# soldasim/BOSS.jl

Measured on AMD Instinct MI355X. Metric: gp_posterior_updates_per_sec (+ acq_evals_per_sec), N=4096 d=8 fp64, higher is better.
Workload: dtype f64; 1 GPU; d=8 synthetic blackbox, GaussianProcess(Matern52) surrogate, N=4096 fp64 posterior update + ExpectedImprovement over 8192 candidates per GPU (BASELINE.json configs[1]+[2]); N=4096, d=8, M_per_gpu=8192, kernel=matern52, parallelism=single GPU: no exchange

## Files before the change

### boss.jl_amd/api.py

```python
from __future__ import annotations

import ctypes as C
import os
from typing import Optional, Sequence

import numpy as np

_HERE = os.path.dirname(os.path.abspath(__file__))
LIB_PATH = os.environ.get("BOSS_LIB_PATH") or os.path.join(_HERE, "libbosship.so")

BOSS_OK, BOSS_E_INVALID, BOSS_E_NO_DEVICE, BOSS_E_NOT_PD, BOSS_E_NEG_VAR, BOSS_E_NOT_FITTED, BOSS_E_ALLOC = range(7)
KERNELS = {"matern32": 0, "matern52": 1, "sqexp": 2}
FIT_NO_SYNC = 1

_c_dp = C.POINTER(C.c_double)
_c_ucp = C.POINTER(C.c_ubyte)

SIGNATURES = {
    "boss_version": (C.c_char_p, []),
    "boss_last_error": (C.c_char_p, []),
    "boss_device_count": (C.c_int, [C.POINTER(C.c_int)]),
    "boss_set_stream": (C.c_int, [C.c_int, C.c_void_p]),
    "boss_device_sync": (C.c_int, [C.c_int]),
    "boss_gp_create": (C.c_int, [C.c_int, C.c_int, C.c_int, C.c_int, _c_dp, _c_dp, _c_ucp, C.POINTER(C.c_void_p)]),
# ... 2283 lines not shown
    return ms.value, n.value


def _update_path(g: GP):
    lib = load_library()
    fn = lib.boss_debug_update_path
    fn.restype = C.c_int
    fn.argtypes = [C.c_void_p, C.POINTER(C.c_int), C.POINTER(C.c_int), C.POINTER(C.c_int)]
    ch, tm, fb = C.c_int(0), C.c_int(0), C.c_int(0)
    _check(fn(g._h, C.byref(ch), C.byref(tm), C.byref(fb)))
    return ch.value, tm.value, fb.value


def _append_path(g: GP) -> int:
    fn = load_library().boss_debug_append_path
    fn.restype = C.c_int
    fn.argtypes = [C.c_void_p, C.POINTER(C.c_int)]
    out = C.c_int(-1)
    _check(fn(g._h, C.byref(out)))
    return out.value


def _fallbacks(device: int = 0):
    lib = load_library()
    fn = lib.boss_debug_fallbacks
    fn.restype = C.c_int
    fn.argtypes = [C.c_int, C.POINTER(C.c_long), C.POINTER(C.c_int)]
    n, off = C.c_long(0), C.c_int(0)
    _check(fn(device, C.byref(n), C.byref(off)))
    return n.value, off.value


def _set_launches(device: int = 0):
    lib = load_library()
    fn = lib.boss_debug_set_launches
    fn.restype = C.c_int
    fn.argtypes = [C.c_int, C.POINTER(C.c_long), C.POINTER(C.c_long)]
    a, b = C.c_long(0), C.c_long(0)
    fn(device, C.byref(a), C.byref(b))
    return a.value, b.value


def _set_grad_launches(device: int = 0):
    lib = load_library()
    fn = lib.boss_debug_set_grad_launches
    fn.restype = C.c_int
    fn.argtypes = [C.c_int, C.POINTER(C.c_long)]
    a = C.c_long(0)
    fn(device, C.byref(a))
    return a.value


def _acq_path(device: int = 0):
    fn = load_library().boss_debug_acq_path
    fn.restype = C.c_int
    fn.argtypes = [C.c_int, C.POINTER(C.c_int)]
    out = (C.c_int * 5)()
    _check(fn(device, out))
    return tuple(out)


def _acq_prune_set(device: int = 0, min_tiles: int = -1, K: int = -1, s: int = -1, cap: int = -1, slack: Optional[float] = None):
    lib = load_library()
    fn = lib.boss_debug_acq_prune_set
    fn.restype = C.c_int
    fn.argtypes = [C.c_int] * 5
    _check(fn(device, int(min_tiles), int(K), int(s), int(cap)))
    if slack is not None:
        fs = lib.boss_debug_acq_prune_slack
        fs.restype = C.c_int
        fs.argtypes = [C.c_int, C.c_double]
        _check(fs(device, float(slack)))


def _acq_prune_bounds(M: int, device: int = 0):
    fn = load_library().boss_debug_acq_prune_bounds
    fn.restype = C.c_int
    fn.argtypes = [C.c_int, C.c_int, C.c_void_p, C.c_void_p, C.c_void_p]
    mua, vs, ub = np.zeros(M), np.zeros(M), np.zeros(M)
    _check(fn(device, int(M), mua.ctypes.data, vs.ctypes.data, ub.ctypes.data))
    return mua, vs, ub


def _acq_counters(g: GP):
    fn = load_library().boss_debug_acq_counters
    fn.restype = C.c_int
    fn.argtypes = [C.c_void_p, C.POINTER(C.c_long)]
    out = (C.c_long * 4)()
    _check(fn(g._h, out))
    return tuple(out)
```

### boss.jl_amd/csrc/bosship.hip

```cpp
#include "../../include/bosship.h"

#include <hip/hip_runtime.h>

#include <algorithm>
#include <cmath>
#include <cstdint>
#include <cstdio>
#include <cstdlib>
#include <atomic>
#include <chrono>
#include <cstring>
#include <functional>
#include <limits>
#include <map>
#include <mutex>
#include <string>
#include <thread>
#include <vector>

#include "gp_kernels.hpp"
#include "potrf.hpp"
#include "chain.hpp"
#include "small_calls.hpp"
#include "rider.hpp"
// ... 409 lines not shown
        hipEvent_t e;
        (void)hipEventCreate(&e);
        return e;
    }
};

struct boss_gpset {
    Ctx* ctx = nullptr;
    std::atomic<int> refs{0};
    void* slab = nullptr;
    void* host_block = nullptr;
    size_t slab_bytes = 0, host_bytes = 0;
};
static bool slab_cache_on() {
    static const bool v = !(getenv("BOSS_SLAB_CACHE") && atoi(getenv("BOSS_SLAB_CACHE")) == 0) &&
                          !poison_alloc();
    return v;
}
static void gpset_release_storage(boss_gpset* st) {
    Ctx* c = st->ctx;
    void *slab = st->slab, *hb = st->host_block;
    if (c && slab_cache_on()) {
        std::lock_guard<std::mutex> lk(c->slab_mtx);
        if (slab && st->slab_bytes > c->slab_cache_bytes) {
            std::swap(slab, c->slab_cache);
            c->slab_cache_bytes = st->slab_bytes;
        }
        if (hb && st->host_bytes > c->hostblk_cache_bytes) {
            std::swap(hb, c->hostblk_cache);
            c->hostblk_cache_bytes = st->host_bytes;
        }
    }
    if (slab) (void)hipFree(slab);
    if (hb) (void)hipHostFree(hb);
    st->slab = st->host_block = nullptr;
}

struct boss_gp {
    Ctx* ctx = nullptr;
    boss_gpset* set = nullptr;
    int kernel = 0, d = 0, N = 0, Np = 0, nblk = 0, ld = 0;
    double *Xraw = nullptr, *Xsc = nullptr, *y = nullptr, *mean = nullptr, *A = nullptr;
    double *LT = nullptr, *DT2 = nullptr, *avec = nullptr;
    bool have_lt = false;
    double *inv16 = nullptr, *Dinv = nullptr, *Dinv2 = nullptr, *hyp = nullptr, *invlam = nullptr, *scal = nullptr;
    int* info = nullptr;
    unsigned char* discrete_dev = nullptr;
    std::vector<unsigned char> discrete;
    double amp2 = 0.0;
    bool has_mean = false, fitted = false, pending = false, have_dinv = false;
    bool dinv_used = false;
    bool dinv_used_prev = false;
    bool gated = false;
    bool chained = false;
    bool fell_back = false;
    int trail_used = -1;
    double* host_res = nullptr;
    double* host_res_dev = nullptr;
    bool par_in_args = false;
    unsigned long long res_seq = 0;
    bool res_polled = false;
    double* host_par = nullptr;
    hipEvent_t par_ev = nullptr;
    unsigned long long epoch = 0;
    unsigned long long factor_gen = 0, dinv0_gen = ~0ull;
    hipEvent_t dinv_ev = nullptr;
    bool dinv_pending = false;
    bool aug = false;
    int npts = 0, ldx = 0, nhead = 0;
    bool gibbs = false;
    double *lamX = nullptr, *ampX = nullptr, *noiseX = nullptr;
    bool kprog = false;
    bool kgrad = false;
    FitProg* kp = nullptr;
    double *Winv = nullptr, *Linv = nullptr;
    double* W2 = nullptr;
    int w2_np = 0;
    unsigned long long w2_gen = ~0ull;
    bool w2_used = false;
    bool have_winv = false;
    int few_calls = 0;
    int append_calls = 0;
    double* prune_a = nullptr;
    int prune_a_np = 0;
    unsigned long long prune_a_gen = ~0ull;
    int prune_skip = 0, prune_backoff = 0;
    int append_path = 0;
};

struct boss_cand {
    Ctx* ctx = nullptr;
    int d = 0, M = 0, Mp = 0;
    double* Craw = nullptr;
};

struct boss_track {
    Ctx* ctx = nullptr;
    boss_gp* gp = nullptr;
    int d = 0, M = 0, Mp = 0, tiles = 0, Ncap = 0, N = 0;
    unsigned long long epoch = 0;
    double *V = nullptr, *Csc = nullptr, *mu = nullptr, *var = nullptr, *mean = nullptr;
    bool has_mean = false;
    bool gibbs = false;
    double *Clam = nullptr, *Camp = nullptr;
    bool aug = false;
};

static inline int round_up(int x, int m) { return (x + m - 1) / m * m; }
struct SetBatch {
    int nb = 1;
    size_t sA = 0, sInv16 = 0, sDinv = 0, sDinv2 = 0, sW = 0, sX = 0;
    size_t sPar = 0;
};
struct MeanFold {
    const double* J = nullptr;
    size_t sJ = 0;
    int T = 0;
    double* dmean = nullptr;
    double* dtheta = nullptr;
};
static void linv_enqueue(boss_gp* g, hipStream_t s, double* U, double* Lw, const SetBatch& B = SetBatch());
constexpr int MAX_ROWS = 46080;

extern "C" const char* boss_version(void) { return "bosship 0.1.0 (gfx950, fp64 MFMA)"; }
extern "C" const char* boss_last_error(void) { return g_last_error.c_str(); }

extern "C" int boss_device_count(int* n_out) {
    const int n = visible_devices();
    hipError_t e = n > 0 ? hipSuccess : hipErrorNoDevice;
    if (e != hipSuccess || n <= 0) {
        if (n_out) *n_out = 0;
        return fail(BOSS_E_NO_DEVICE, "no HIP device visible (bosship has no CPU fallback)");
    }
    if (n_out) *n_out = n;
    return BOSS_OK;
}

extern "C" int boss_set_stream(int device, void* hip_stream) {
    Ctx* c;
    int rc = get_ctx(device, &c);
    if (rc) return rc;
    std::lock_guard<std::mutex> lk(c->mtx);
    HIPCHK(hipStreamSynchronize(c->stream));
    c->stream = hip_stream ? (hipStream_t)hip_stream : c->own_stream;
    return BOSS_OK;
}

extern "C" int boss_device_sync(int device) {
    Ctx* c;
    int rc = get_ctx(device, &c);
    if (rc) return rc;
    HIPCHK(hipStreamSynchronize(c->stream));
    return BOSS_OK;
}

static bool few_done_ensure(Ctx* c, hipStream_t s) {
    if (c->few_done) return true;
    if (hipMalloc((void**)&c->few_done, sizeof(unsigned long long)) != hipSuccess) {
        (void)hipGetLastError();
        c->few_done = nullptr;
        return false;
    }
    (void)hipMemsetAsync(c->few_done, 0, sizeof(unsigned long long), s);
    c->few_done_cnt = 0;
    return true;
}
// ... 181 lines not shown
```

### boss.jl_amd/csrc/host_factor.inc

```


struct LaunchStamps {
    static constexpr int CAP = 512;
    int n = 0;
    int tag[CAP];
    std::chrono::steady_clock::time_point t[CAP];
    void reset() { n = 0; }
    void add(int what) {
        if (n < CAP) {
            tag[n] = what;
            t[n++] = std::chrono::steady_clock::now();
        }
    }
};
static std::atomic<int> g_stamps_on{-1};
static std::atomic<long long> g_stall_us{2500};
static std::mutex g_stall_mtx;
static std::string g_stall_log;
static bool launch_stamps_on() {
    int v = g_stamps_on.load(std::memory_order_relaxed);
    if (v < 0) {
        v = (getenv("BOSS_LAUNCH_STAMPS") && atoi(getenv("BOSS_LAUNCH_STAMPS"))) ? 1 : 0;
        if (getenv("BOSS_STALL_MS")) g_stall_us.store((long long)(atof(getenv("BOSS_STALL_MS")) * 1000.0));
        g_stamps_on.store(v);
// ... 394 lines not shown
        if (m == 0) {
            if (step_hook && chain_inline) (*step_hook)(k);
            break;
        }
        if (la && (m <= small_m + 1 || chain)) {
            const bool poll = last_rest >= 0 && last_rest == tail_join && bulk_pub != 0;
            if (last_rest >= 0 && !poll) (void)hipStreamWaitEvent(s, c->ev_rest[last_rest], 0);
            last_rest = -1;
            if (chain_inline && plan->tab) {
                const int* off = plan->tab_off;
                hipLaunchKernelGGL(potrf_colupd_tab_kernel, dim3(off[k + 1] - off[k]), dim3(256), 0, s, A, ld, plan->tab + off[k], k, critw);
            } else
                hipLaunchKernelGGL(potrf_colupd_kernel, dim3(2 * m * (m + 1) + m, 1, batch), dim3(256), 0, s, A, ld, bstride, k,
                                   m, m, 0, 1, poll ? c->sig_panel + bulk_pub_word : (unsigned long long*)nullptr, bulk_pub, info, chain ? 1 : 0, -1, critw, budget);
            BOSS_STAMP(2000 + k);
            if (step_hook && chain_inline) (*step_hook)(k);
            continue;
        }
        if (!la) {
            ProfScope ps(c, "potrf_syrk");
            hipLaunchKernelGGL(potrf_syrk_kernel<1>, dim3(m * (m + 1) / 2 + m, 1, batch), dim3(256), 0, s, A, ld, bstride, k,
                               k + 1, m, 0);
            continue;
        }
        {
            const bool poll = last_rest >= 0 && last_rest == tail_join && bulk_pub != 0;
            if (last_rest >= 0 && !poll) (void)hipStreamWaitEvent(s, c->ev_rest[last_rest], 0);
            hipLaunchKernelGGL(potrf_colupd_kernel, dim3(4 * m + 1, 1, batch), dim3(256), 0, s, A, ld, bstride, k, m, 1, 0, 1,
                               poll ? c->sig_panel + bulk_pub_word : (unsigned long long*)nullptr, bulk_pub, info, 0, -1, (unsigned long long*)nullptr, budget);
        }
        last_rest = -1;
#ifdef BOSS_EXPERIMENTS
        static const int exp_norest = getenv("BOSS_EXP_NOREST") ? atoi(getenv("BOSS_EXP_NOREST")) : 0;
#else
        constexpr int exp_norest = 0;
#endif
        if (m >= 2 && exp_norest != 1) {
            const int m2 = m - 1;
            (void)hipEventRecord(c->ev_panel[k], s);
            (void)hipStreamWaitEvent(c->side_stream, c->ev_panel[k], 0);
            if (exp_norest != 2)
                hipLaunchKernelGGL(potrf_syrk_kernel<1>, dim3(m2 * (m2 + 1) / 2 + m2, 1, batch), dim3(256), 0, c->side_stream, A,
                                   ld, bstride, k, k + 2, m2, 0);
            (void)hipEventRecord(c->ev_rest[k], c->side_stream);
            last_rest = k;
        }
    }
    if (la && last_rest >= 0) (void)hipStreamWaitEvent(s, c->ev_rest[last_rest], 0);
}

static void gram_enqueue(Ctx* c, const double* Xsc, size_t xs_bstride, int d, int N, int Np, int kern,
                         const double* hyp, double* A, int ld, size_t bstride, int batch) {
    ProfScope ps(c, "gram");
    const int nt = Np / 64;
    hipLaunchKernelGGL(gram_kernel, dim3(nt * (nt + 1) / 2, 1, batch), dim3(256), 0, c->stream, Xsc, xs_bstride, d, N,
                       Np, kern, hyp, A, ld, bstride, 0);
}

static void gp_release(boss_gp* g) {
    if (!g) return;
    if (g->ctx) (void)hipSetDevice(g->ctx->device);
    if (g->ctx) chain_quiesce(g->ctx);
    if (g->set) {
        if (g->ctx) (void)hipStreamSynchronize(g->ctx->stream);
        if (g->dinv_pending && g->ctx) (void)hipStreamSynchronize(g->ctx->side_stream);
        boss_gpset* st = g->set;
        if (st->refs.fetch_sub(1) == 1) {
            gpset_release_storage(st);
            delete st;
        }
        g->Xraw = g->Xsc = g->y = g->mean = g->A = g->inv16 = g->Dinv = g->Dinv2 = g->invlam = g->scal = nullptr;
        g->lamX = g->ampX = g->noiseX = nullptr;
        g->host_res = g->host_par = nullptr;
        g->set = nullptr;
    }
    void* ptrs[] = {g->Xraw, g->Xsc, g->y, g->mean, g->A, g->inv16, g->Dinv, g->Dinv2, g->LT, g->DT2, g->avec, g->invlam, g->scal, g->discrete_dev};
    for (void* p : ptrs)
        if (p) (void)hipFree(p);
    if (g->host_res) (void)hipHostFree(g->host_res);
    if (g->Winv) (void)hipFree(g->Winv);
    if (g->Linv) (void)hipFree(g->Linv);
    if (g->W2) (void)hipFree(g->W2);
    if (g->prune_a) (void)hipFree(g->prune_a);
    if (g->lamX) (void)hipFree(g->lamX);
    if (g->ampX) (void)hipFree(g->ampX);
    if (g->noiseX) (void)hipFree(g->noiseX);
    if (g->host_par) (void)hipHostFree(g->host_par);
    delete g->kp;
    if (g->par_ev) (void)hipEventDestroy(g->par_ev);
    if (g->dinv_ev) (void)hipEventDestroy(g->dinv_ev);
    delete g;
}

static void pack_points(std::vector<double>& dst, const double* X, int d, int n, int ldp,
                        const unsigned char* discrete) {
    dst.assign((size_t)d * ldp, 0.0);
    for (int j = 0; j < n; ++j)
        for (int k = 0; k < d; ++k) {
            double v = X[(size_t)j * d + k];
            if (discrete && discrete[k]) v = std::nearbyint(v);
            dst[(size_t)k * ldp + j] = v;
        }
}

static int gp_create_common(int device, int kernel, int d, int npts, int N, const double* X, const double* y,
                            const unsigned char* discrete, bool aug, boss_gp_t** out) {
    if (!out) return fail(BOSS_E_INVALID, "out is NULL");
    *out = nullptr;
    if (kernel < 0 || kernel > 2) return fail(BOSS_E_INVALID, "unknown kernel id");
    if (d < 1 || N < 1 || !X || !y) return fail(BOSS_E_INVALID, "need d >= 1, N >= 1 and non-NULL X, y");
    if (N > MAX_ROWS) return fail(BOSS_E_INVALID, "more than 46080 rows (observations, or n (1 + d) with gradients) are not supported");
    Ctx* c;
    int rc = get_ctx(device, &c);
    if (rc) return rc;
    boss_gp* g = new boss_gp();
    g->ctx = c;
    g->kernel = kernel;
    g->d = d;
    g->N = N;
    g->Np = round_up(N, PRED_RB);
    g->nblk = g->Np / BLK;
    g->ld = g->Np + RHS_ROWS;
    g->aug = aug;
    g->npts = npts;
    g->nhead = npts;
    g->ldx = aug ? round_up(npts, 64) : g->Np;
    const size_t Np = g->Np, ldx = g->ldx;
#define GALLOC(ptr, bytes)                                        \
    do {                                                          \
        hipError_t e_ = dev_malloc((void**)&(ptr), (bytes));       \
        if (e_ != hipSuccess) {                                   \
            gp_release(g);                                        \
            return fail(BOSS_E_ALLOC, "device allocation failed"); \
        }                                                         \
    } while (0)
    GALLOC(g->Xraw, sizeof(double) * d * ldx);
    GALLOC(g->Xsc, sizeof(double) * d * ldx);
    GALLOC(g->y, sizeof(double) * Np);
    GALLOC(g->mean, sizeof(double) * Np);
    GALLOC(g->A, sizeof(double) * (size_t)g->ld * Np);
    GALLOC(g->inv16, sizeof(double) * g->nblk * 8 * 256);
    GALLOC(g->Dinv, sizeof(double) * g->nblk * BLK * BLK);
    GALLOC(g->Dinv2, sizeof(double) * (g->Np / PRED_RB) * PRED_RB * PRED_RB);
    GALLOC(g->invlam, sizeof(double) * (d + 4));
    g->hyp = g->invlam + d;
    GALLOC(g->scal, sizeof(double) * 4);
    g->info = (int*)(g->scal + 2);
    if (hipHostMalloc((void**)&g->host_res, 512, hipHostMallocDefault) != hipSuccess ||
        hipHostMalloc((void**)&g->host_par, sizeof(double) * (d + 4), hipHostMallocDefault) != hipSuccess ||
        hipEventCreateWithFlags(&g->par_ev, hipEventDisableTiming) != hipSuccess ||
        hipEventCreateWithFlags(&g->dinv_ev, hipEventDisableTiming) != hipSuccess ||
        hipHostGetDevicePointer((void**)&g->host_res_dev, g->host_res, 0) != hipSuccess) {
        gp_release(g);
        return fail(BOSS_E_ALLOC, "pinned allocation failed");
    }
    std::memset(g->host_res, 0, 512);
    if (discrete) {
        g->discrete.assign(discrete, discrete + d);
        bool any = false;
        for (int k = 0; k < d; ++k) any |= discrete[k] != 0;
        if (any) {
            GALLOC(g->discrete_dev, d);
            (void)hipMemcpy(g->discrete_dev, discrete, d, hipMemcpyHostToDevice);
        } else {
            g->discrete.clear();
        }
// ... 559 lines not shown
```

### boss.jl_amd/csrc/host_prune.inc

```

struct PruneCfg {
    int min_tiles = -1;
    int K = 64;
    int s = 1;
    int cap = 1024;
    double slack = 1.0;
};
static PruneCfg g_prune;
constexpr double PRUNE_KMU = 1.2e-4, PRUNE_KVAR = 1e-10;
constexpr size_t PRUNE_RES_OFF = 16;

static bool prune_enabled() {
    static const bool on = !(getenv("BOSS_ACQ_PRUNE") && atoi(getenv("BOSS_ACQ_PRUNE")) == 0);
    static const bool once = [] {
        if (getenv("BOSS_ACQ_PRUNE_BLOCKS")) g_prune.s = std::max(1, atoi(getenv("BOSS_ACQ_PRUNE_BLOCKS")));
        if (getenv("BOSS_ACQ_PRUNE_CAP")) g_prune.cap = std::max(0, atoi(getenv("BOSS_ACQ_PRUNE_CAP")));
        return true;
    }();
    (void)once;
    return on;
}

extern "C" int boss_debug_acq_path(int device, int* out) {
    if (!out) return fail(BOSS_E_INVALID, "out is NULL");
    Ctx* c;
    int rc = get_ctx(device, &c);
    if (rc) return rc;
    std::lock_guard<std::mutex> lk(c->mtx);
    for (int i = 0; i < 5; ++i) out[i] = c->prune_last[i];
    return BOSS_OK;
}
extern "C" int boss_debug_acq_prune_set(int device, int min_tiles, int K, int s, int cap) {
    (void)device;
    (void)prune_enabled();
    const PruneCfg def;
    if (min_tiles != -1) g_prune.min_tiles = min_tiles < -1 ? def.min_tiles : min_tiles;
    if (K != -1) g_prune.K = K < 1 ? def.K : K;
    if (s != -1) g_prune.s = s < 1 ? def.s : s;
    if (cap != -1) g_prune.cap = cap < -1 ? def.cap : cap;
    return BOSS_OK;
}
extern "C" int boss_debug_acq_counters(const boss_gp* g, long* out) {
    if (!g || !out) return fail(BOSS_E_INVALID, "NULL argument");
    out[0] = g->have_winv ? 1 : 0;
    out[1] = g->few_calls;
    out[2] = g_dev_allocs.load();
    out[3] = g->ctx->prune_launches;
    return BOSS_OK;
}
extern "C" int boss_debug_acq_prune_slack(int device, double scale) {
    (void)device;
    if (!(scale >= 0.0)) return fail(BOSS_E_INVALID, "scale must be >= 0");
    g_prune.slack = scale;
    return BOSS_OK;
}
extern "C" int boss_debug_acq_prune_bounds(int device, int M, double* mua_out, double* vars_out, double* ub_out) {
    Ctx* c;
    int rc = get_ctx(device, &c);
    if (rc) return rc;
    std::lock_guard<std::mutex> lk(c->mtx);
    if (M < 1 || M != c->prune_M || !c->prunews.p) return fail(BOSS_E_INVALID, "no pruned attempt with that many candidates");
    HIPCHK(hipStreamSynchronize(c->stream));
    const double* base = (const double*)c->prunews.p;
    if (mua_out) HIPCHK(hipMemcpy(mua_out, base, sizeof(double) * M, hipMemcpyDeviceToHost));
    if (vars_out) HIPCHK(hipMemcpy(vars_out, base + M, sizeof(double) * M, hipMemcpyDeviceToHost));
    if (ub_out) HIPCHK(hipMemcpy(ub_out, base + 2 * (size_t)M, sizeof(double) * M, hipMemcpyDeviceToHost));
    return BOSS_OK;
}

static bool prune_eligible(const boss_gp* g, const boss_cand* cd, int P, int S, const EiPar& par, bool has_out, bool defer, bool has_mc,
                           const double* dpair) {
    if (!prune_enabled() || has_out || defer || dpair || has_mc || P != 1 || S != 1 || par.mode != 1) return false;
    if (g->aug || g->gibbs || g->kprog || g->ctx->prof_on) return false;
    const int ftiles = (cd->M + 31) / 32;
    const int min_tiles = g_prune.min_tiles >= 0 ? g_prune.min_tiles : few_max_tiles();
    if (few_off() || ftiles <= min_tiles || g->Np < 4 * PRED_RB || g->d > 64 || cd->d != g->d || slab_bn(cd->M, false) != 32) return false;
    if (small_predict_ok(g, cd->M) || cd->M <= g_prune.K || cd->M > PRUNE_THREADS * PRUNE_CPT_MAX) return false;
    if (g_prune.K > 32 * few_max_tiles()) return false;
    return g_prune.s < g->Np / PRED_RB;
}

static bool prune_poll(Ctx* c, hipStream_t s, const double* res, unsigned long long want) {
    volatile const unsigned long long* seq = reinterpret_cast<volatile const unsigned long long*>(res) + 4;
    bool got = false;
    for (unsigned long i = 1;; ++i) {
        if (*seq == want) {
            got = true;
            break;
        }
        if ((i & 0x3fff) == 0 && hipStreamQuery(s) != hipErrorNotReady) break;
    }
    std::atomic_thread_fence(std::memory_order_acquire);
    if (!got) {
        (void)hipStreamSynchronize(s);
        got = *seq == want;
    }
    return got;
}

static int prune_avec(boss_gp* g, hipStream_t s, const double** a_out, bool* rebuilt) {
    *rebuilt = false;
    if (g->have_lt && g->avec) {
        *a_out = g->avec;
        return BOSS_OK;
    }
    if (g->prune_a && g->prune_a_np != g->Np) {
        (void)hipStreamSynchronize(s);
        (void)hipFree(g->prune_a);
        g->prune_a = nullptr;
    }
    if (!g->prune_a) {
        if (dev_malloc((void**)&g->prune_a, sizeof(double) * 2 * (size_t)g->Np) != hipSuccess) {
            g->prune_a = nullptr;
            return fail(BOSS_E_ALLOC, "device allocation failed");
        }
        g->prune_a_np = g->Np;
        g->prune_a_gen = ~0ull;
    }
    if (g->prune_a_gen != g->factor_gen) {
        const int nb = g->Np / PRED_RB;
        for (int ib = nb - 1; ib >= 0; --ib)
            hipLaunchKernelGGL(prune_avec_step_kernel, dim3(std::max(1, 2 * ib)), dim3(PRUNE_AVEC_THREADS), 0, s, (const double*)g->A, g->ld, g->Np, g->N,
                               (const double*)g->Dinv2, ib, ib == nb - 1 ? 1 : 0, g->prune_a + g->Np, g->prune_a);
        g->prune_a_gen = g->factor_gen;
        *rebuilt = true;
    }
    *a_out = g->prune_a;
    return BOSS_OK;
}

static int acq_prune_try(boss_gp* g, const boss_cand* cd, const double* mean_dev, const unsigned char* mask_dev, const EiPar& par,
                         bool* done, double* res_out, long* idx_out) {
    *done = false;
    Ctx* c = g->ctx;
    hipStream_t s = c->stream;
    int* last = c->prune_last;
    last[0] = 0;
    last[1] = last[2] = last[4] = 0;
    last[3] = g_prune.s;
    if (g->prune_skip > 0) {
        --g->prune_skip;
        last[0] = 3;
        return BOSS_OK;
    }
    const int M = cd->M, Mp = cd->Mp, d = g->d, Np = g->Np, nch = Np / PRUNE_MU_ROWS, sblk = g_prune.s, K = g_prune.K;
    const int cap = std::min(g_prune.cap, 32 * few_max_tiles()), tiles = (M + 31) / 32;
    const size_t nint = (size_t)round_up(std::max(K, cap), 64);
    const size_t nd = (size_t)4 * M + (size_t)nch * M + 3 * nint + (size_t)d * nint + 2;
    int rc = ws_reserve(c->prunews, sizeof(double) * nd + sizeof(int) * (nint + (size_t)M) + (size_t)M);
    if (rc) return rc;
    rc = ws_reserve(c->csc, sizeof(double) * (size_t)d * Mp);
    if (rc) return rc;
    rc = ws_reserve(c->vscratch, sizeof(double) * (size_t)tiles * 32 * Np);
    if (rc) return rc;
    double* mua = (double*)c->prunews.p;
    double* vars = mua + M;
    double* ub = vars + M;
    unsigned long long* keys = (unsigned long long*)(ub + M);
    double* part = ub + 2 * (size_t)M;
    double* imu = part + (size_t)nch * M;
    double* ivar = imu + nint;
    double* imean = ivar + nint;
    double* icraw = imean + nint;
    double* tpair = icraw + (size_t)d * nint;
    int* sel = (int*)(tpair + 2);
    int* surv = sel + nint;
    unsigned char* insel = (unsigned char*)(surv + M);
    c->prune_M = M;
    double* res = (double*)c->pinned + PRUNE_RES_OFF;

    if (!g->have_dinv) {
        dinv_join(g);
        dinv_launch(g, s);
        g->have_dinv = true;
    }
    dinv_join(g);
    g->dinv_used = true;
    const double* avec = nullptr;
    bool rebuilt = false;
    rc = prune_avec(g, s, &avec, &rebuilt);
    if (rc) return rc;
    last[4] = rebuilt ? 1 : 0;
    c->prune_launches += (rebuilt ? Np / PRED_RB : 0) + 7;
    double* Csc = (double*)c->csc.p;
    hipLaunchKernelGGL(scale_cand_kernel, dim3((Mp + 255) / 256), dim3(256), 0, s, cd->Craw, Csc, g->invlam, g->discrete_dev, d, Mp);
    typedef PredG32 G;
    hipLaunchKernelGGL(prune_head_kernel<G>, dim3(tiles), dim3(G::NTHREADS), PredictLds<G>::BYTES, s, (const double*)g->A, g->ld, Np, g->N,
                       (const double*)g->Dinv2, (const double*)g->Xsc, (const double*)Csc, d, Mp, g->kernel, g->amp2, (double*)c->vscratch.p, M,
                       sblk, vars);
    const size_t mu_lds = sizeof(double) * ((size_t)d + 1) * PRUNE_MU_STAGE;
    auto mu_fn = d <= 16 ? prune_mu_kernel<true> : prune_mu_kernel<false>;
    hipLaunchKernelGGL(mu_fn, dim3((M + PRUNE_MU_CANDS - 1) / PRUNE_MU_CANDS, nch), dim3(256), mu_lds, s, (const double*)g->Xsc, Np, g->N, (const double*)Csc, d, Mp, M,
                       g->kernel, g->amp2, avec, part);
    PrunePar pp;
    pp.coef = par.coefs[0];
    pp.best = par.best;
    pp.amp2 = g->amp2;
    pp.kmu = PRUNE_KMU * g_prune.slack;
    pp.kvar = PRUNE_KVAR * g_prune.slack;
    hipLaunchKernelGGL(prune_bound_kernel, dim3((M + 255) / 256), dim3(256), 0, s, (const double*)part, nch, mean_dev, (const double*)vars, mask_dev, M,
                       pp, mua, ub, keys);
    hipLaunchKernelGGL(prune_select_kernel, dim3(1), dim3(PRUNE_THREADS), 0, s, (const unsigned long long*)keys, M, K, sel, insel);

    boss_cand icd;
    icd.ctx = c;
    icd.d = d;
    auto finish_exact = [&](const int* list, int n) -> int {
        icd.M = n;
        icd.Mp = round_up(n, 64);
        icd.Craw = icraw;
        hipLaunchKernelGGL(prune_gather_kernel, dim3((icd.Mp + 255) / 256), dim3(256), 0, s, list, n, (const double*)cd->Craw, Mp, d, mean_dev,
                           icraw, icd.Mp, mean_dev ? imean : (double*)nullptr);
        return predict_enqueue(g, &icd, mean_dev ? imean : nullptr, imu, ivar, false, nullptr, nullptr, false, true);
    };
    rc = finish_exact(sel, K);
    if (rc) return drain(c, rc);
    unsigned long long seq = ++c->acq_seq;
    hipLaunchKernelGGL(prune_decide_kernel, dim3(1), dim3(PRUNE_THREADS), 0, s, (const int*)sel, K, (const double*)imu, (const double*)ivar,
                       (const double*)mua, mask_dev, par, pp, M, (const double*)ub, (const unsigned char*)insel, surv, tpair, res, seq);
    bool ok = prune_poll(c, s, res, seq);
    hipError_t e = hipGetLastError();
    if (!ok || e != hipSuccess) return fail(BOSS_E_NO_DEVICE, e != hipSuccess ? hipGetErrorString(e) : "the pruned acquisition did not report");
    long cnt = reinterpret_cast<const long*>(res)[2], bad = reinterpret_cast<const long*>(res)[3];
    last[1] = K;
    last[2] = (int)std::min<long>(cnt, 0x7fffffff);
    if (!bad && cnt > 0 && cnt <= cap) {
        rc = finish_exact(surv, (int)cnt);
        if (rc) return drain(c, rc);
        c->prune_launches += 2;
        seq = ++c->acq_seq;
        hipLaunchKernelGGL(prune_merge_kernel, dim3(1), dim3(PRUNE_THREADS), 0, s, (const int*)surv, (int)cnt, (const double*)imu,
                           (const double*)ivar, (const double*)mua, mask_dev, par, pp, (const double*)tpair, res, seq);
        ok = prune_poll(c, s, res, seq);
        e = hipGetLastError();
        if (!ok || e != hipSuccess) return fail(BOSS_E_NO_DEVICE, e != hipSuccess ? hipGetErrorString(e) : "the pruned acquisition did not report");
        bad = reinterpret_cast<const long*>(res)[3];
    }
    if (bad || cnt > cap) {
        g->prune_backoff = g->prune_backoff ? std::min(64, 2 * g->prune_backoff) : 1;
        g->prune_skip = g->prune_backoff;
        last[0] = 2;
        return BOSS_OK;
    }
    g->prune_backoff = 0;
    last[0] = 1;
    *res_out = res[0];
    *idx_out = reinterpret_cast<const long*>(res)[1];
    *done = true;
    return BOSS_OK;
}
```

### boss.jl_amd/csrc/prune_kernels.hpp

```cpp
#pragma once
#include "acq_kernels.hpp"

namespace boss {

template <int NC>
__device__ __forceinline__ void prune_wave_sums(double (&v)[NC], int lane) {
#pragma unroll
    for (int h = NC / 2; h >= 1; h >>= 1) {
        const bool up = (lane & h) != 0;
#pragma unroll
        for (int j = 0; j < h; ++j) {
            const double keep = up ? v[j + h] : v[j], send = up ? v[j] : v[j + h];
            v[j] = keep + __shfl_xor(send, h);
        }
    }
#pragma unroll
    for (int off = NC; off < 64; off <<= 1) v[0] += __shfl_xor(v[0], off);
}
constexpr int PRUNE_AVEC_THREADS = 1024;
__global__ __launch_bounds__(PRUNE_AVEC_THREADS) void prune_avec_step_kernel(const double* __restrict__ A, int ld, int Np, int N,
                                                                             const double* __restrict__ Dinv2, int ib, int first,
                                                                             double* __restrict__ r, double* __restrict__ a) {
    __shared__ double rv[PRED_RB], av[PRED_RB];
    const int tid = threadIdx.x, lane = tid & 63;
    const int wave = __builtin_amdgcn_readfirstlane(tid >> 6);
    const int i0 = ib * PRED_RB;
    if (tid < PRED_RB) {
        const int i = i0 + tid;
        rv[tid] = first ? (i < N ? A[(size_t)i * ld + Np] : 0.0) : r[i];
    }
    __syncthreads();
    const double* D = Dinv2 + (size_t)ib * PRED_RB * PRED_RB;
    double r4[4];
#pragma unroll
    for (int q = 0; q < 4; ++q) r4[q] = rv[lane + 64 * q];
    {
        double sums[16];
#pragma unroll
        for (int j = 0; j < 16; ++j) {
            const int c = 16 * j + wave;
            const double* col = D + (size_t)c * PRED_RB;
            double sacc = 0.0;
#pragma unroll
            for (int q = 0; q < 4; ++q) {
                if (q >= j / 4) {
                    const int row = lane + 64 * q;
                    const double dv = col[row];
                    sacc = __builtin_fma(row >= c ? dv : 0.0, r4[q], sacc);
                }
            }
            sums[j] = sacc;
        }
        prune_wave_sums<16>(sums, lane);
        if (lane < 16) av[16 * lane + wave] = sums[0];
    }
    __syncthreads();
    if (blockIdx.x == 0 && tid < PRED_RB) a[i0 + tid] = av[tid];
    if (ib == 0) return;
    double a4[4];
#pragma unroll
    for (int q = 0; q < 4; ++q) a4[q] = av[lane + 64 * q];
    double sums[8];
    const int cg0 = blockIdx.x * 128 + wave * 8;
#pragma unroll
    for (int j = 0; j < 8; ++j) {
        const double* col = A + (size_t)(cg0 + j) * ld + i0;
        double sacc = 0.0;
#pragma unroll
        for (int q = 0; q < 4; ++q) sacc = __builtin_fma(col[lane + 64 * q], a4[q], sacc);
        sums[j] = sacc;
    }
    prune_wave_sums<8>(sums, lane);
    if (lane < 8) {
        const int cg = cg0 + lane;
        const double base = first ? (cg < N ? A[(size_t)cg * ld + Np] : 0.0) : r[cg];
        r[cg] = base - sums[0];
    }
}

template <class G>
__global__ __launch_bounds__(G::NTHREADS) __attribute__((amdgpu_waves_per_eu(1, 1))) void prune_head_kernel(
    const double* __restrict__ A, int ld, int Np, int N, const double* __restrict__ Dinv, const double* __restrict__ Xsc,
    const double* __restrict__ Csc, int d, int Mp, int kern, double amp2, double* __restrict__ Vscratch, int M, int sblk,
    double* __restrict__ var_out) {
    static_assert(G::WC == 1 && G::BM == 2 * BLK && G::PM == 2 && G::WR == 4, "written for the 256-row, 32-candidate geometry");
    constexpr int RB = G::BM;
    extern __shared__ double lds[];
    constexpr int BN = G::BN, TM = G::TM, TN = G::TN, LDR = PredictLds<G>::LDR;
    double* Rs = lds;
    double* red = Rs + RB * LDR;
    const int tid = threadIdx.x, lane = tid & 63;
    const int wave = __builtin_amdgcn_readfirstlane(tid >> 6);
    const int wr = wave, wc = 0;
    const int tile = blockIdx.x, c0 = tile * BN;
    double* V = Vscratch + (size_t)tile * sblk * RB * BN;
    double* part = red + 2 * G::WR * G::BN;
#pragma unroll
    for (int u = 0; u < TN * 4; ++u) part[u * G::NTHREADS + tid] = 0.0;
    double* cs = part + (size_t)G::NTHREADS * PredictLds<G>::PART;
    const bool cs_ok = d <= PRED_CS_MAX_D;
    if (cs_ok) {
        for (int idx = tid; idx < d * BN; idx += G::NTHREADS) cs[idx] = Csc[(size_t)(idx / BN) * Mp + c0 + (idx % BN)];
        __syncthreads();
    }
    for (int ib = 0; ib < sblk; ++ib) {
        v4d acc[TM][TN];
#pragma unroll
        for (int m = 0; m < TM; ++m)
#pragma unroll
            for (int n = 0; n < TN; ++n) acc[m][n] = v4d{0.0, 0.0, 0.0, 0.0};
        G::template run<1>(A + (size_t)ib * RB, ld, V, BN, ib * RB, acc);
        double r2[TM][TN][4];
#pragma unroll
        for (int m = 0; m < TM; ++m)
#pragma unroll
            for (int n = 0; n < TN; ++n)
#pragma unroll
                for (int i = 0; i < 4; ++i) r2[m][n][i] = 0.0;
        if (cs_ok) {
            for (int kd0 = 0; kd0 < d; kd0 += 4) {
                double xr[4][TM];
#pragma unroll
                for (int kk = 0; kk < 4; ++kk)
#pragma unroll
                    for (int m = 0; m < TM; ++m)
                        xr[kk][m] = (kd0 + kk < d) ? Xsc[(size_t)(kd0 + kk) * Np + ib * RB + G::row_of(wr, m, lane)] : 0.0;
#pragma unroll
                for (int kk = 0; kk < 4; ++kk) {
                    if (kd0 + kk < d) {
#pragma unroll
                        for (int n = 0; n < TN; ++n)
#pragma unroll
                            for (int i = 0; i < 4; ++i) {
                                const double xc = cs[(kd0 + kk) * BN + G::col_of(wc, n, i, lane)];
#pragma unroll
                                for (int m = 0; m < TM; ++m) {
                                    const double diff = xr[kk][m] - xc;
                                    r2[m][n][i] = __builtin_fma(diff, diff, r2[m][n][i]);
                                }
                            }
                    }
                }
            }
        } else
        for (int kd = 0; kd < d; ++kd) {
            double xr[TM], xc[TN][4];
#pragma unroll
            for (int m = 0; m < TM; ++m) xr[m] = Xsc[(size_t)kd * Np + ib * RB + G::row_of(wr, m, lane)];
#pragma unroll
            for (int n = 0; n < TN; ++n)
#pragma unroll
                for (int i = 0; i < 4; ++i) xc[n][i] = Csc[(size_t)kd * Mp + c0 + G::col_of(wc, n, i, lane)];
#pragma unroll
            for (int m = 0; m < TM; ++m)
#pragma unroll
                for (int n = 0; n < TN; ++n)
#pragma unroll
                    for (int i = 0; i < 4; ++i) {
                        double diff = xr[m] - xc[n][i];
                        r2[m][n][i] = __builtin_fma(diff, diff, r2[m][n][i]);
// ... 407 lines not shown
```

Measured before the change: 918.1 updates/s.

## Precompute block coupling matrices to shorten the serial chain of the prune a-vector solve

```diff
diff --git a/boss.jl_amd/api.py b/boss.jl_amd/api.py
--- a/boss.jl_amd/api.py
+++ b/boss.jl_amd/api.py
@@ -2389,6 +2389,15 @@
     return mua, vs, ub
 
 
+def _acq_avec(g: GP):
+    fn = load_library().boss_debug_acq_avec
+    fn.restype = C.c_int
+    fn.argtypes = [C.c_void_p, C.c_void_p, C.c_int]
+    a = np.zeros(g.N)
+    _check(fn(g._h, a.ctypes.data, int(g.N)))
+    return a
+
+
 def _acq_counters(g: GP):
     fn = load_library().boss_debug_acq_counters
     fn.restype = C.c_int
diff --git a/boss.jl_amd/csrc/bosship.hip b/boss.jl_amd/csrc/bosship.hip
--- a/boss.jl_amd/csrc/bosship.hip
+++ b/boss.jl_amd/csrc/bosship.hip
@@ -515,6 +515,7 @@
     int few_calls = 0;
     int append_calls = 0;
     double* prune_a = nullptr;
+    double* prune_u = nullptr;
     int prune_a_np = 0;
     unsigned long long prune_a_gen = ~0ull;
     int prune_skip = 0, prune_backoff = 0;
diff --git a/boss.jl_amd/csrc/host_factor.inc b/boss.jl_amd/csrc/host_factor.inc
--- a/boss.jl_amd/csrc/host_factor.inc
+++ b/boss.jl_amd/csrc/host_factor.inc
@@ -500,6 +500,7 @@
     if (g->Linv) (void)hipFree(g->Linv);
     if (g->W2) (void)hipFree(g->W2);
     if (g->prune_a) (void)hipFree(g->prune_a);
+    if (g->prune_u) (void)hipFree(g->prune_u);
     if (g->lamX) (void)hipFree(g->lamX);
     if (g->ampX) (void)hipFree(g->ampX);
     if (g->noiseX) (void)hipFree(g->noiseX);
diff --git a/boss.jl_amd/csrc/host_prune.inc b/boss.jl_amd/csrc/host_prune.inc
--- a/boss.jl_amd/csrc/host_prune.inc
+++ b/boss.jl_amd/csrc/host_prune.inc
@@ -68,6 +68,16 @@
     return BOSS_OK;
 }
 
+extern "C" int boss_debug_acq_avec(const boss_gp* g, double* out, int n) {
+    if (!g || !out) return fail(BOSS_E_INVALID, "NULL argument");
+    if (!g->prune_a || g->prune_a_gen != g->factor_gen || n < 1 || n > g->Np) return fail(BOSS_E_INVALID, "no current a = L^-T z of the chain");
+    HIPCHK(hipSetDevice(g->ctx->device));
+    std::lock_guard<std::mutex> lk(g->ctx->mtx);
+    HIPCHK(hipStreamSynchronize(g->ctx->stream));
+    HIPCHK(hipMemcpy(out, g->prune_a, sizeof(double) * n, hipMemcpyDeviceToHost));
+    return BOSS_OK;
+}
+
 static bool prune_eligible(const boss_gp* g, const boss_cand* cd, int P, int S, const EiPar& par, bool has_out, bool defer, bool has_mc,
                            const double* dpair) {
     if (!prune_enabled() || has_out || defer || dpair || has_mc || P != 1 || S != 1 || par.mode != 1) return false;
@@ -104,24 +114,34 @@
         *a_out = g->avec;
         return BOSS_OK;
     }
-    if (g->prune_a && g->prune_a_np != g->Np) {
+    const int nb = g->Np / PRED_RB;
+    if ((g->prune_a || g->prune_u) && g->prune_a_np != g->Np) {
         (void)hipStreamSynchronize(s);
-        (void)hipFree(g->prune_a);
-        g->prune_a = nullptr;
-    }
-    if (!g->prune_a) {
-        if (dev_malloc((void**)&g->prune_a, sizeof(double) * 2 * (size_t)g->Np) != hipSuccess) {
+        if (g->prune_a) (void)hipFree(g->prune_a);
+        if (g->prune_u) (void)hipFree(g->prune_u);
+        g->prune_a = g->prune_u = nullptr;
+    }
+    if (!g->prune_a || !g->prune_u) {
+        g->prune_a_np = g->Np;
+        g->prune_a_gen = ~0ull;
+        if (!g->prune_a && dev_malloc((void**)&g->prune_a, sizeof(double) * 2 * (size_t)g->Np) != hipSuccess) {
             g->prune_a = nullptr;
             return fail(BOSS_E_ALLOC, "device allocation failed");
         }
-        g->prune_a_np = g->Np;
-        g->prune_a_gen = ~0ull;
+        if (!g->prune_u && dev_malloc((void**)&g->prune_u, sizeof(double) * (size_t)(nb - 1) * PRED_RB * PRED_RB) != hipSuccess) {
+            g->prune_u = nullptr;
+            return fail(BOSS_E_ALLOC, "device allocation failed");
+        }
     }
     if (g->prune_a_gen != g->factor_gen) {
-        const int nb = g->Np / PRED_RB;
-        for (int ib = nb - 1; ib >= 0; --ib)
-            hipLaunchKernelGGL(prune_avec_step_kernel, dim3(std::max(1, 2 * ib)), dim3(PRUNE_AVEC_THREADS), 0, s, (const double*)g->A, g->ld, g->Np, g->N,
-                               (const double*)g->Dinv2, ib, ib == nb - 1 ? 1 : 0, g->prune_a + g->Np, g->prune_a);
+        double* r = g->prune_a + g->Np;
+        hipLaunchKernelGGL(prune_u_kernel, dim3(PRED_RB / PRUNE_U_COLS, nb - 1), dim3(PRUNE_U_THREADS), 0, s, (const double*)g->A, g->ld, g->Np, g->N,
+                           (const double*)g->Dinv2, g->prune_u, r);
+        for (int ib = nb - 1; ib >= 0; --ib) {
+            const bool last = ib == nb - 1;
+            hipLaunchKernelGGL(prune_avec_step_kernel, dim3(PRUNE_CRIT_WGS + (last ? 0 : ib * (PRED_RB / PRUNE_UPD_COLS))), dim3(PRUNE_AVEC_THREADS), 0, s,
+                               (const double*)g->A, g->ld, (const double*)g->Dinv2, (const double*)g->prune_u, ib, last ? 1 : 0, r, g->prune_a);
+        }
         g->prune_a_gen = g->factor_gen;
         *rebuilt = true;
     }
@@ -181,7 +201,7 @@
     rc = prune_avec(g, s, &avec, &rebuilt);
     if (rc) return rc;
     last[4] = rebuilt ? 1 : 0;
-    c->prune_launches += (rebuilt ? Np / PRED_RB : 0) + 7;
+    c->prune_launches += (rebuilt ? Np / PRED_RB + 1 : 0) + 7;
     double* Csc = (double*)c->csc.p;
     hipLaunchKernelGGL(scale_cand_kernel, dim3((Mp + 255) / 256), dim3(256), 0, s, cd->Craw, Csc, g->invlam, g->discrete_dev, d, Mp);
     typedef PredG32 G;
diff --git a/boss.jl_amd/csrc/prune_kernels.hpp b/boss.jl_amd/csrc/prune_kernels.hpp
--- a/boss.jl_amd/csrc/prune_kernels.hpp
+++ b/boss.jl_amd/csrc/prune_kernels.hpp
@@ -17,65 +17,152 @@
 #pragma unroll
     for (int off = NC; off < 64; off <<= 1) v[0] += __shfl_xor(v[0], off);
 }
-constexpr int PRUNE_AVEC_THREADS = 1024;
-__global__ __launch_bounds__(PRUNE_AVEC_THREADS) void prune_avec_step_kernel(const double* __restrict__ A, int ld, int Np, int N,
-                                                                             const double* __restrict__ Dinv2, int ib, int first,
-                                                                             double* __restrict__ r, double* __restrict__ a) {
-    __shared__ double rv[PRED_RB], av[PRED_RB];
+constexpr int PRUNE_U_COLS = 8, PRUNE_U_THREADS = PRED_RB / 2, PRUNE_U_KB = 16;
+__device__ __forceinline__ void prune_u_steps(const double2 (&l)[PRUNE_U_KB], const double* __restrict__ dk, double2 (&acc)[PRUNE_U_COLS]) {
+#pragma unroll
+    for (int kk = 0; kk < PRUNE_U_KB; ++kk)
+#pragma unroll
+        for (int j = 0; j < PRUNE_U_COLS; ++j) {
+            const double d = dk[kk * PRUNE_U_COLS + j];
+            acc[j].x = __builtin_fma(l[kk].x, d, acc[j].x);
+            acc[j].y = __builtin_fma(l[kk].y, d, acc[j].y);
+        }
+}
+__global__ __launch_bounds__(PRUNE_U_THREADS) void prune_u_kernel(const double* __restrict__ A, int ld, int Np, int N,
+                                                                  const double* __restrict__ Dinv2, double* __restrict__ U,
+                                                                  double* __restrict__ r) {
+    static_assert(PRED_RB % PRUNE_U_COLS == 0 && PRED_RB % PRUNE_U_KB == 0 && PRUNE_U_THREADS * (PRED_RB / PRUNE_U_COLS) >= 2 * PRED_RB,
+                  "the grid's threads cover the Np entries of r");
+    constexpr int KB = PRUNE_U_KB;
+    __shared__ double Ds[PRED_RB * PRUNE_U_COLS];
+    const int ib = blockIdx.y, c0 = blockIdx.x * PRUNE_U_COLS, t = threadIdx.x;
+    const int gi = (blockIdx.y * gridDim.x + blockIdx.x) * PRUNE_U_THREADS + t;
+    if (gi < Np) r[gi] = gi < N ? A[(size_t)gi * ld + Np] : 0.0;
+    const double* D = Dinv2 + (size_t)ib * PRED_RB * PRED_RB + (size_t)c0 * PRED_RB;
+    const int kbeg = c0 & ~(KB - 1);
+    const size_t cs = (size_t)ld / 2;
+    const double2* Lb = reinterpret_cast<const double2*>(A + (size_t)ib * PRED_RB * ld + (size_t)(ib + 1) * PRED_RB) + t;
+    double2 la[KB], lb[KB];
+#pragma unroll
+    for (int kk = 0; kk < KB; ++kk) la[kk] = Lb[(size_t)(kbeg + kk) * cs];
+#pragma unroll
+    for (int j = 0; j < PRUNE_U_COLS; ++j)
+#pragma unroll
+        for (int h = 0; h < PRED_RB / PRUNE_U_THREADS; ++h) {
+            const int k = t + h * PRUNE_U_THREADS;
+            const double v = D[(size_t)j * PRED_RB + k];
+            Ds[k * PRUNE_U_COLS + j] = k >= c0 + j ? v : 0.0;
+        }
+    double2 acc[PRUNE_U_COLS];
+#pragma unroll
+    for (int j = 0; j < PRUNE_U_COLS; ++j) acc[j] = double2{0.0, 0.0};
+    __syncthreads();
+    for (int k0 = kbeg; k0 < PRED_RB; k0 += 2 * KB) {
+#pragma unroll
+        for (int kk = 0; kk < KB; ++kk) lb[kk] = Lb[(size_t)min(k0 + KB + kk, PRED_RB - 1) * cs];
+        prune_u_steps(la, Ds + k0 * PRUNE_U_COLS, acc);
+        if (k0 + KB >= PRED_RB) break;
+#pragma unroll
+        for (int kk = 0; kk < KB; ++kk) la[kk] = Lb[(size_t)min(k0 + 2 * KB + kk, PRED_RB - 1) * cs];
+        prune_u_steps(lb, Ds + (k0 + KB) * PRUNE_U_COLS, acc);
+    }
+    double2* Uo = reinterpret_cast<double2*>(U + (size_t)ib * PRED_RB * PRED_RB + (size_t)c0 * PRED_RB) + t;
+#pragma unroll
+    for (int j = 0; j < PRUNE_U_COLS; ++j) Uo[(size_t)j * (PRED_RB / 2)] = acc[j];
+}
+
+constexpr int PRUNE_AVEC_THREADS = 512, PRUNE_AVEC_WAVES = PRUNE_AVEC_THREADS / 64;
+constexpr int PRUNE_CRIT_COLS = 16, PRUNE_UPD_COLS = 32;
+constexpr int PRUNE_CRIT_WGS = PRED_RB / PRUNE_CRIT_COLS;
+constexpr int PRUNE_CRIT_CPW = PRUNE_CRIT_COLS / PRUNE_AVEC_WAVES, PRUNE_UPD_CPW = PRUNE_UPD_COLS / PRUNE_AVEC_WAVES;
+static_assert(PRUNE_CRIT_CPW >= 1 && PRUNE_UPD_CPW >= 1 && (PRED_RB / 2) % PRUNE_CRIT_COLS == 0, "whole columns per wave; a critical "
+              "workgroup's columns lie in one half of the block");
+template <bool LOW, bool HAS_U>
+__device__ __forceinline__ void prune_crit_shares(const double2* __restrict__ D, const double2* __restrict__ Ub,
+                                                  const double2* __restrict__ rv, const double2* __restrict__ av, int cb, int lane,
+                                                  double (&sums)[PRUNE_CRIT_CPW]) {
+    constexpr int H = PRED_RB / 2 / 2;
+    double2 dl[PRUNE_CRIT_CPW], dh[PRUNE_CRIT_CPW], ul[PRUNE_CRIT_CPW], uh[PRUNE_CRIT_CPW];
+    const double2 zero = {0.0, 0.0};
+#pragma unroll
+    for (int j = 0; j < PRUNE_CRIT_CPW; ++j) {
+        dl[j] = LOW ? D[(size_t)j * 2 * H + lane] : zero;
+        dh[j] = D[(size_t)j * 2 * H + H + lane];
+        ul[j] = HAS_U ? Ub[(size_t)j * 2 * H + lane] : zero;
+        uh[j] = HAS_U ? Ub[(size_t)j * 2 * H + H + lane] : zero;
+    }
+    const double2 rl = LOW ? rv[lane] : zero, rh = rv[H + lane];
+    const double2 al = HAS_U ? av[lane] : zero, ah = HAS_U ? av[H + lane] : zero;
+    const int r0 = 2 * lane, r1 = PRED_RB / 2 + 2 * lane;
+#pragma unroll
+    for (int j = 0; j < PRUNE_CRIT_CPW; ++j) {
+        const int c = cb + j;
+        double s = 0.0;
+        if (LOW) {
+            s = __builtin_fma(r0 >= c ? dl[j].x : 0.0, rl.x, s);
+            s = __builtin_fma(r0 + 1 >= c ? dl[j].y : 0.0, rl.y, s);
+        }
+        s = __builtin_fma(r1 >= c ? dh[j].x : 0.0, rh.x, s);
+        s = __builtin_fma(r1 + 1 >= c ? dh[j].y : 0.0, rh.y, s);
+        if (HAS_U) {
+            double t = ul[j].x * al.x;
+            t = __builtin_fma(ul[j].y, al.y, t);
+            t = __builtin_fma(uh[j].x, ah.x, t);
+            t = __builtin_fma(uh[j].y, ah.y, t);
+            s -= t;
+        }
+        sums[j] = s;
+    }
+}
+__global__ __launch_bounds__(PRUNE_AVEC_THREADS) void prune_avec_step_kernel(const double* __restrict__ A, int ld,
+                                                                             const double* __restrict__ Dinv2,
+                                                                             const double* __restrict__ U, int ib, int last,
+                                                                             double* r, double* a) {
     const int tid = threadIdx.x, lane = tid & 63;
     const int wave = __builtin_amdgcn_readfirstlane(tid >> 6);
     const int i0 = ib * PRED_RB;
-    if (tid < PRED_RB) {
-        const int i = i0 + tid;
-        rv[tid] = first ? (i < N ? A[(size_t)i * ld + Np] : 0.0) : r[i];
-    }
-    __syncthreads();
-    const double* D = Dinv2 + (size_t)ib * PRED_RB * PRED_RB;
-    double r4[4];
-#pragma unroll
-    for (int q = 0; q < 4; ++q) r4[q] = rv[lane + 64 * q];
-    {
-        double sums[16];
-#pragma unroll
-        for (int j = 0; j < 16; ++j) {
-            const int c = 16 * j + wave;
-            const double* col = D + (size_t)c * PRED_RB;
-            double sacc = 0.0;
-#pragma unroll
-            for (int q = 0; q < 4; ++q) {
-                if (q >= j / 4) {
-                    const int row = lane + 64 * q;
-                    const double dv = col[row];
-                    sacc = __builtin_fma(row >= c ? dv : 0.0, r4[q], sacc);
-                }
-            }
-            sums[j] = sacc;
-        }
-        prune_wave_sums<16>(sums, lane);
-        if (lane < 16) av[16 * lane + wave] = sums[0];
-    }
-    __syncthreads();
-    if (blockIdx.x == 0 && tid < PRED_RB) a[i0 + tid] = av[tid];
-    if (ib == 0) return;
-    double a4[4];
-#pragma unroll
-    for (int q = 0; q < 4; ++q) a4[q] = av[lane + 64 * q];
-    double sums[8];
-    const int cg0 = blockIdx.x * 128 + wave * 8;
-#pragma unroll
-    for (int j = 0; j < 8; ++j) {
-        const double* col = A + (size_t)(cg0 + j) * ld + i0;
-        double sacc = 0.0;
-#pragma unroll
-        for (int q = 0; q < 4; ++q) sacc = __builtin_fma(col[lane + 64 * q], a4[q], sacc);
-        sums[j] = sacc;
-    }
-    prune_wave_sums<8>(sums, lane);
-    if (lane < 8) {
-        const int cg = cg0 + lane;
-        const double base = first ? (cg < N ? A[(size_t)cg * ld + Np] : 0.0) : r[cg];
-        r[cg] = base - sums[0];
-    }
+    if (blockIdx.x < PRUNE_CRIT_WGS) {
+        const int cb = blockIdx.x * PRUNE_CRIT_COLS + wave * PRUNE_CRIT_CPW;
+        const size_t off = (size_t)ib * PRED_RB * PRED_RB + (size_t)cb * PRED_RB;
+        const double2* D = reinterpret_cast<const double2*>(Dinv2 + off);
+        const double2* Ub = reinterpret_cast<const double2*>(U + off);
+        const double2* rv = reinterpret_cast<const double2*>(r + i0);
+        const double2* av = reinterpret_cast<const double2*>(a + i0 + PRED_RB);
+        const bool low = blockIdx.x * PRUNE_CRIT_COLS < PRED_RB / 2;
+        double sums[PRUNE_CRIT_CPW];
+        if (last) {
+            if (low) prune_crit_shares<true, false>(D, Ub, rv, av, cb, lane, sums);
+            else prune_crit_shares<false, false>(D, Ub, rv, av, cb, lane, sums);
+        } else {
+            if (low) prune_crit_shares<true, true>(D, Ub, rv, av, cb, lane, sums);
+            else prune_crit_shares<false, true>(D, Ub, rv, av, cb, lane, sums);
+        }
+        prune_wave_sums<PRUNE_CRIT_CPW>(sums, lane);
+        if (lane < PRUNE_CRIT_CPW) a[i0 + cb + lane] = sums[0];
+        return;
+    }
+    constexpr int H = PRED_RB / 2 / 2;
+    const int cg0 = (blockIdx.x - PRUNE_CRIT_WGS) * PRUNE_UPD_COLS + wave * PRUNE_UPD_CPW;
+    const double2* av = reinterpret_cast<const double2*>(a + i0 + PRED_RB);
+    double2 ll[PRUNE_UPD_CPW], lh[PRUNE_UPD_CPW];
+#pragma unroll
+    for (int j = 0; j < PRUNE_UPD_CPW; ++j) {
+        const double2* col = reinterpret_cast<const double2*>(A + (size_t)(cg0 + j) * ld + i0 + PRED_RB);
+        ll[j] = col[lane];
+        lh[j] = col[H + lane];
+    }
+    const double2 al = av[lane], ah = av[H + lane];
+    double sums[PRUNE_UPD_CPW];
+#pragma unroll
+    for (int j = 0; j < PRUNE_UPD_CPW; ++j) {
+        double t = ll[j].x * al.x;
+        t = __builtin_fma(ll[j].y, al.y, t);
+        t = __builtin_fma(lh[j].x, ah.x, t);
+        t = __builtin_fma(lh[j].y, ah.y, t);
+        sums[j] = t;
+    }
+    prune_wave_sums<PRUNE_UPD_CPW>(sums, lane);
+    if (lane < PRUNE_UPD_CPW) r[cg0 + lane] -= sums[0];
 }
 
 template <class G>
```

Result: no change. 915.6 updates/s (-0.3%).
